# smithlabcode/walt

Hardware: AMD Instinct MI355X
Metric: mapped reads/sec (100 bp single-end, hg19-scale index, -m 6 -b 5000) (higher is better)
Workload: dtype u32

## Files before the change

walt_amd/csrc/core.h:

```cpp
#ifndef WALT_AMD_CORE_H_
#define WALT_AMD_CORE_H_

#include <stdint.h>
#if !defined(__HIPCC__)
#include <stdio.h>
#include <stdlib.h>
#endif

#if defined(__HIPCC__)
#define WALT_HD __host__ __device__ __forceinline__
#else
#define WALT_HD inline
#endif

namespace walt {

#ifndef WALT_SEEDPATTERN
#define WALT_SEEDPATTERN 3
#endif
static_assert(WALT_SEEDPATTERN == 3 || WALT_SEEDPATTERN == 5 || WALT_SEEDPATTERN == 7, "seed pattern 3, 5 or 7");
constexpr uint32_t kPat = WALT_SEEDPATTERN;
constexpr uint32_t kCareW = kPat == 3 ? 1 : (kPat == 5 ? 2 : 4);
constexpr uint32_t kNoCareW = kPat - kCareW;
constexpr uint32_t kKeyWeight = 12;
// ... 1180 lines not shown
  q_of.start_index = iv.start_index; q_of.n_chrom = iv.n_chrom;
  seed_lookup_ex(iv, sv, care, slot, span, seed_len, out, known_good, q_of);
}

WALT_HD Region seed_lookup(const IndexView& iv, const StrandView& sv, const uint32_t* care, uint32_t slot,
                           uint32_t span, uint32_t seed_len) {
  Lookup lk;
  seed_lookup_ex(iv, sv, care, slot, span, seed_len, lk);
  return lk.reg;
}

WALT_HD uint32_t popc32(uint32_t x) {
#if defined(__HIP_DEVICE_COMPILE__)
  return __popc(x);
#else
  return (uint32_t)__builtin_popcount(x);
#endif
}
WALT_HD uint32_t funnel_r(uint32_t lo, uint32_t hi, uint32_t s) {
#if defined(__HIP_DEVICE_COMPILE__)
  return __funnelshift_r(lo, hi, s);
#else
  return (uint32_t)((((uint64_t)hi << 32) | lo) >> s);
#endif
}

constexpr uint32_t tail_care_base_word(uint32_t w) {
  uint32_t m = 0;
  for (uint32_t p = kKeyWeight + kKeyChars; p < kNumCare; ++p) {
    const uint32_t o = care_pos(p);
    if ((o >> 4) == w) m |= 1u << (2 * (o & 15u));
  }
  return m;
}
WALT_HD uint32_t tail_mask_word(uint32_t w, uint32_t lo, uint32_t hi);
template <int W>
WALT_HD uint32_t tail_care_mask_word(uint32_t seed_i, uint32_t cut) {
  constexpr uint32_t b1 = tail_care_base_word(W), b0 = W ? tail_care_base_word(W ? W - 1 : 0) : 0u;
  const uint32_t s = 2 * seed_i;
  const uint32_t m = (b1 << s) | (s ? b0 >> (32 - s) : 0u);
  return m & tail_mask_word(W, 0, cut);
}
WALT_HD uint32_t tail_care_cut(uint32_t seed_i, uint32_t seed_len) {
  return seed_len < kNumCare ? seed_i + care_pos(seed_len) : 0xFFFFu;
}

template <int NW>
WALT_HD uint32_t count_mismatch(const uint32_t* g2, uint32_t gpos, const uint32_t* rd, const uint32_t* mask) {
  const uint32_t* g = g2 + (gpos >> 4);
  uint32_t sh = 2 * (gpos & 15);
  uint32_t mm = 0;
  uint32_t cur = g[0];
#pragma unroll
  for (int w = 0; w < NW; ++w) {
    uint32_t nxt = g[w + 1];
    uint32_t x = funnel_r(cur, nxt, sh) ^ rd[w];
    mm += popc32((x | (x >> 1)) & mask[w]);
    cur = nxt;
  }
  return mm;
}

template <int NW, int W = 0>
WALT_HD void count_mismatch_tail_words(const uint32_t* g, uint32_t sh, const uint32_t* rd, const uint32_t* mask,
                                       uint32_t seed_i, uint32_t cut, uint32_t cur, uint32_t& mm, uint32_t& tmm) {
  if constexpr (W < NW) {
    const uint32_t nxt = g[W + 1];
    const uint32_t x = funnel_r(cur, nxt, sh) ^ rd[W];
    const uint32_t d = x | (x >> 1);
    mm += popc32(d & mask[W]);
    tmm += popc32(d & tail_care_mask_word<W>(seed_i, cut));
    count_mismatch_tail_words<NW, W + 1>(g, sh, rd, mask, seed_i, cut, nxt, mm, tmm);
  }
}
template <int NW>
WALT_HD uint32_t count_mismatch_tail(const uint32_t* g2, uint32_t gpos, const uint32_t* rd, const uint32_t* mask,
                                     uint32_t seed_i, uint32_t cut, uint32_t& tmm) {
  const uint32_t* g = g2 + (gpos >> 4);
  uint32_t mm = 0;
  tmm = 0;
  count_mismatch_tail_words<NW>(g, 2 * (gpos & 15), rd, mask, seed_i, cut, g[0], mm, tmm);
  return mm;
}

template <int NW>
WALT_HD uint32_t count_mismatch_regs(const uint32_t* g , uint32_t sh, const uint32_t* rd, const uint32_t* mask) {
  uint32_t mm = 0;
#if defined(__HIP_DEVICE_COMPILE__)
#pragma unroll
#endif
  for (int w = 0; w < NW; ++w) {
    uint32_t x = funnel_r(g[w], g[w + 1], sh) ^ rd[w];
    mm += popc32((x | (x >> 1)) & mask[w]);
  }
  return mm;
}

template <int NW>
WALT_HD uint32_t count_mismatch_regs2(const uint32_t* g , uint32_t sh, const uint32_t* rd, const uint32_t* mask,
                                      const uint32_t* tmask, uint32_t& tmm) {
  uint32_t mm = 0, t = 0;
#if defined(__HIP_DEVICE_COMPILE__)
#pragma unroll
#endif
  for (int w = 0; w < NW; ++w) {
    const uint32_t x = funnel_r(g[w], g[w + 1], sh) ^ rd[w];
    const uint32_t d = x | (x >> 1);
    mm += popc32(d & mask[w]);
    t += popc32(d & tmask[w]);
  }
  tmm = t;
  return mm;
}

WALT_HD uint32_t align_word(uint32_t cur, uint32_t below, uint32_t sh) {
  return (cur << sh) | ((below >> 1) >> (31u - sh));
}
template <int NW>
WALT_HD void align_read(const uint32_t* rd, const uint32_t* mk, uint32_t sh, uint32_t* rd_a , uint32_t* mk_a ) {
  rd_a[0] = align_word(rd[0], 0u, sh);
  mk_a[0] = align_word(mk[0], 0u, sh);
#if defined(__HIP_DEVICE_COMPILE__)
#pragma unroll
#endif
  for (int w = 1; w < NW; ++w) {
    rd_a[w] = align_word(rd[w], rd[w - 1], sh);
    mk_a[w] = align_word(mk[w], mk[w - 1], sh);
  }
  rd_a[NW] = align_word(0u, rd[NW - 1], sh);
  mk_a[NW] = align_word(0u, mk[NW - 1], sh);
}
template <int NW>
WALT_HD uint32_t count_mismatch_aligned(const uint32_t* g , const uint32_t* rd_a, const uint32_t* mk_a, bool top) {
  uint32_t mm = 0;
#if defined(__HIP_DEVICE_COMPILE__)
#pragma unroll
#endif
  for (int w = 0; w < NW; ++w) {
    const uint32_t x = g[w] ^ rd_a[w];
    mm += popc32((x | (x >> 1)) & mk_a[w]);
  }
  if (top) {
    const uint32_t x = g[NW] ^ rd_a[NW];
    mm += popc32((x | (x >> 1)) & mk_a[NW]);
  }
  return mm;
}
template <int NW>
WALT_HD uint32_t aligned_header_word(uint32_t i, uint32_t cur, uint32_t below, uint32_t sh) {
  const bool first = i == 8u || i == 8u + NW;
  return align_word(cur, first ? 0u : below, i >= 8u ? sh : 0u);
}
WALT_HD uint32_t aligned_header_top(uint32_t last, uint32_t sh) { return align_word(0u, last, sh); }

WALT_HD uint32_t care_mask_word(uint32_t w, uint32_t seed_i, uint32_t p0, uint32_t p1) {
  uint32_t m = 0;
  for (uint32_t p = p0; p < p1; ++p) {
    const uint32_t o = seed_i + care_pos(p);
    if ((o >> 4) == w) m |= 1u << (2 * (o & 15u));
  }
  return m;
}

WALT_HD uint32_t tail_mask_word(uint32_t w, uint32_t lo, uint32_t hi) {
  uint32_t b0 = 16 * w, b1 = b0 + 16;
  uint32_t a = lo > b0 ? lo : b0;
  uint32_t b = hi < b1 ? hi : b1;
  if (a >= b) return 0;
  uint32_t na = a - b0, nb = b - b0;
  uint32_t m = nb == 16 ? 0x55555555u : ((1u << (2 * nb)) - 1u) & 0x55555555u;
  uint32_t below = ((1u << (2 * na)) - 1u);
  return m & ~below;
}
WALT_HD uint32_t mask_table_index(uint32_t seed_i, uint32_t repeats, uint32_t w) {
  return (seed_i * (kMaxRepeats - kMinRepeats + 1) + (repeats - kMinRepeats)) * kMaskWords + w;
}
WALT_HD uint32_t compare_mask_word(const uint32_t* mask_table, uint32_t seed_i, uint32_t repeats,
                                   uint32_t read_len, uint32_t w) {
  uint32_t t = w < kMaskWords ? mask_table[mask_table_index(seed_i, repeats, w)] : 0u;
  return t | tail_mask_word(w, kPat * repeats + seed_i, read_len);
}

struct RegionSummary {
  uint32_t min_mm;
  uint32_t count;
  uint32_t first;
  uint32_t last;
};
WALT_HD RegionSummary summary_empty() { RegionSummary s; s.min_mm = 0xFFFFFFFFu; s.count = 0; s.first = 0; s.last = 0; return s; }
WALT_HD RegionSummary summary_one(uint32_t mm, uint32_t pos) { RegionSummary s; s.min_mm = mm; s.count = 1; s.first = pos; s.last = pos; return s; }
WALT_HD RegionSummary summary_merge(const RegionSummary& a, const RegionSummary& b) {
  const bool has_a = a.count != 0, has_b = b.count != 0;
  const bool take_a = has_a && (!has_b || a.min_mm <= b.min_mm);
  const bool take_b = has_b && (!has_a || b.min_mm <= a.min_mm);
  RegionSummary s;
  s.min_mm = take_a ? a.min_mm : b.min_mm;
  s.count = (take_a ? a.count : 0u) + (take_b ? b.count : 0u);
  s.first = take_a ? a.first : b.first;
  s.last = take_b ? b.last : a.last;
  return s;
}
WALT_HD void fold_region(BestMatch& best, const RegionSummary& s, uint32_t strand_char) {
  if (s.count == 0) return;
  if (s.min_mm < best.mismatch) {
    best.genome_pos = s.last; best.times = s.count; best.strand = strand_char; best.mismatch = s.min_mm;
  } else if (s.min_mm == best.mismatch) {
    uint32_t same = (s.first == best.genome_pos) ? 1u : 0u;
    if (s.count > same) {
      best.times += s.count - same;
      best.genome_pos = s.last;
      best.strand = strand_char;
    }
  }
}

struct HeapEnt {
  uint32_t pos, mms;
};
WALT_HD uint32_t heap_mm(const HeapEnt& e) { return e.mms & 0x7FFFFFFFu; }

template <class H>
WALT_HD void heap_sift_up(H h, uint32_t hole, uint32_t top, HeapEnt v) {
  while (hole > top) {
    uint32_t parent = (hole - 1) / 2;
    if (!(heap_mm(h[parent]) < heap_mm(v))) break;
    h[hole] = h[parent];
    hole = parent;
  }
  h[hole] = v;
}
template <class H>
WALT_HD void heap_push(H h, uint32_t& size, HeapEnt v) {
  heap_sift_up(h, size, 0, v);
  ++size;
}
template <class H>
WALT_HD void heap_adjust(H h, uint32_t hole, uint32_t len, HeapEnt v) {
  const uint32_t top = hole;
  uint32_t child = hole;
  while ((int32_t)child < ((int32_t)len - 1) / 2) {
    child = 2 * (child + 1);
    if (heap_mm(h[child]) < heap_mm(h[child - 1])) --child;
    h[hole] = h[child];
    hole = child;
  }
  if ((len & 1) == 0 && (int32_t)child == ((int32_t)len - 2) / 2) {
    child = 2 * (child + 1);
    h[hole] = h[child - 1];
    hole = child - 1;
  }
  heap_sift_up(h, hole, top, v);
}
template <class H>
WALT_HD HeapEnt heap_pop(H h, uint32_t& size) {
  HeapEnt topv = h[0];
  if (size > 1) {
    HeapEnt v = h[size - 1];
    h[size - 1] = topv;
    heap_adjust(h, 0, size - 1, v);
  }
  --size;
  return topv;
}
template <class H>
WALT_HD void topk_push(H h, uint32_t& size, uint32_t k, HeapEnt v) {
  if (size < k) {
    heap_push(h, size, v);
  } else if (heap_mm(v) < heap_mm(h[0])) {
    heap_pop(h, size);
    heap_push(h, size, v);
  }
}

struct Candidate {
  uint32_t genome_pos;
  uint32_t strand;
  uint32_t mismatch;
};
struct PairResult {
  BestMatch m1, m2;
  uint32_t best_times;
  int32_t frag_len;
  int32_t best_i, best_j;
  uint32_t pair_mm;
  uint32_t pad_[3];
};

WALT_HD void forward_pos(uint32_t gp, uint32_t strand_char, uint32_t chr, uint32_t read_len,
                         const uint32_t* start_index, uint32_t& s, uint32_t& e) {
  uint32_t len = start_index[chr + 1] - start_index[chr];
  uint32_t v = gp - start_index[chr];
  s = strand_char == '+' ? v : len - v - read_len;
  e = s + read_len;
}
WALT_HD void best4single(const Candidate* r, int n, BestMatch& best) {
  for (int i = n - 1; i >= 0; --i) {
    if (r[i].mismatch < best.mismatch) {
      best.genome_pos = r[i].genome_pos; best.times = 1; best.strand = r[i].strand; best.mismatch = r[i].mismatch;
    } else if (r[i].mismatch == best.mismatch) {
      if (best.genome_pos == r[i].genome_pos) continue;
      best.genome_pos = r[i].genome_pos; best.strand = r[i].strand; best.times++;
    } else {
      break;
    }
  }
}
// ... 61 lines not shown
```

walt_amd/csrc/map_se.hip:

```cpp
#include <stdio.h>
#include <stdlib.h>
#include <string.h>

#include "map_common.h"
#include "map_items.h"
#include "group_core.h"

namespace walt {

static __global__ __launch_bounds__(kBlock) void k_ascii_to_2bit(const uint8_t* __restrict__ bases,
                                                                  const uint64_t* __restrict__ offsets, uint32_t n,
                                                                  uint32_t* __restrict__ codes2, uint64_t cap_bytes,
                                                                  uint32_t* __restrict__ err) {
  const uint64_t o0 = offsets[0], all = offsets[n] - o0, total = all < cap_bytes ? all : cap_bytes;
  if (all > cap_bytes && blockIdx.x == 0 && threadIdx.x == 0) atomicAdd(err + 1, 1u);
  const uint8_t* src = bases + o0;
  const uint32_t mis = (uint32_t)(reinterpret_cast<uintptr_t>(src) & 15);
  const uint64_t nwords = (total + 15) / 16;
  uint32_t bad_total = 0;
  for (uint64_t i = (uint64_t)blockIdx.x * blockDim.x + threadIdx.x; i < nwords;
       i += (uint64_t)gridDim.x * blockDim.x) {
    uint32_t qs[4] = {0, 0, 0, 0};
    const uint64_t b0 = 16 * i;
    if (mis == 0 && b0 + 16 <= total) {
// ... 1393 lines not shown
__device__ __forceinline__ const uint4* share_item(const HeavyStage& hs, uint32_t i, uint32_t n_big) {
  constexpr uint32_t Q = item_quads<NW>();
  return i < n_big ? hs.giants + (uint64_t)Q * i : hs.items + (uint64_t)Q * (i - n_big);
}
__device__ __forceinline__ unsigned long long wave_sum_u64(unsigned long long v) {
#pragma unroll
  for (int off = 32; off > 0; off >>= 1) v += __shfl_xor(v, off);
  return v;
}

template <int NW, bool SCATTER>
__global__ __launch_bounds__(kBlock) void k_se_share_bin(HeavyStage hs, SeShare sh) {
  uint32_t n_big, n_all;
  share_counts(hs, n_big, n_all);
  const uint32_t n_grp = n_all < sh.cap ? n_all : sh.cap;
  unsigned long long beyond = 0;
  for (uint32_t i = blockIdx.x * blockDim.x + threadIdx.x; i < (SCATTER ? n_grp : n_all); i += gridDim.x * blockDim.x) {
    const uint4 h = load_global(share_item<NW>(hs, i, n_big));
    if (i < n_grp) {
      const uint32_t bk = group_bucket(group_key(h.x, h.w));
      if constexpr (SCATTER) {
        const uint32_t at = atomicAdd(&sh.cursor[bk], 1u);
        if (at < sh.cap) sh.order[at] = i;
      } else {
        atomicAdd(&sh.count[bk], 1u);
      }
    } else {
      beyond += h.z;
    }
  }
  if constexpr (!SCATTER) {
    if (n_all > n_grp) {
      beyond = wave_sum_u64(beyond);
      if ((threadIdx.x & 63) == 0 && beyond) {
        atomicAdd(&sh.recs[0], beyond);
        atomicAdd(&sh.recs[1], beyond);
      }
    }
  }
}

constexpr uint32_t kShareScanThreads = 1024;
__global__ __launch_bounds__(kShareScanThreads) void k_se_share_scan(SeShare sh) {
  constexpr uint32_t per = kGroupBuckets / kShareScanThreads;
  __shared__ uint32_t part[kShareScanThreads];
  const uint32_t t = threadIdx.x;
  uint32_t s = 0;
  for (uint32_t k = 0; k < per; ++k) s += sh.count[t * per + k];
  part[t] = s;
  __syncthreads();
  for (uint32_t off = 1; off < kShareScanThreads; off <<= 1) {
    const uint32_t v = t >= off ? part[t - off] : 0u;
    __syncthreads();
    part[t] += v;
    __syncthreads();
  }
  uint32_t run = part[t] - s;
  for (uint32_t k = 0; k < per; ++k) {
    sh.cursor[t * per + k] = run;
    run += sh.count[t * per + k];
    sh.count[t * per + k] = 0u;
  }
}

template <int NW>
__global__ __launch_bounds__(kBlock) void k_se_share_cut(HeavyStage hs, SeShare sh) {
  uint32_t n_big, n_all;
  share_counts(hs, n_big, n_all);
  const uint32_t lane = threadIdx.x & 63;
  const uint32_t n_waves = (gridDim.x * blockDim.x) >> 6, wave = (blockIdx.x * blockDim.x + threadIdx.x) >> 6;
  const uint32_t r = sh.r ? sh.r : 1u;
  unsigned long long rec_items = 0, rec_units = 0;
  uint32_t rode = 0;
  const uint32_t end = n_all < sh.cap ? n_all : sh.cap;
  for (uint32_t s = wave * kGroupSlice; s < end; s += n_waves * kGroupSlice) {
    const uint32_t p = s + lane;
    const bool valid = p < end;
    uint32_t item = sh.order[valid ? p : s];
    item = item < n_all ? item : 0u;
    const uint4* it = share_item<NW>(hs, item, n_big);
    const uint4 h0 = load_global(it), h1 = load_global(it + 1);
    const uint64_t key = group_key(h0.x, h0.w);
    const uint32_t size = h0.z, tail = h1.z;
    unsigned long long rem = __ballot(valid);
    uint32_t placed = 0;
    GroupPlace mine = {0u, 0u, 1u, true};
    while (rem) {
      const int ld = (int)__ffsll((long long)rem) - 1;
      const uint64_t lkey = group_key(bcast(h0.x, ld), bcast(h0.w, ld));
      const bool join = (int)lane == ld || group_joins(key, size, tail, lkey, bcast(size, ld), bcast(tail, ld));
      const unsigned long long m = __ballot(join) & rem;
      if ((m >> lane) & 1ull) mine = group_place(m, lane, placed, r);
      placed += (uint32_t)__popcll(m);
      rem &= ~m;
    }
    if (valid) sh.order[s + mine.pos] = item;
    const bool leads = valid && mine.leads, big = size > kBigFirst;
    const unsigned long long mb = __ballot(leads && big), mr = __ballot(leads && !big);
    uint32_t base_b = 0, base_r = 0;
    if (lane == 0) {
      if (mb) base_b = atomicAdd(&sh.ctl[0], (uint32_t)__popcll(mb));
      if (mr) base_r = atomicAdd(&sh.ctl[1], (uint32_t)__popcll(mr));
    }
    base_b = bcast(base_b, 0);
    base_r = bcast(base_r, 0);
    if (leads) {
      const unsigned long long below = (1ull << lane) - 1ull;
      const uint32_t k = big ? base_b + (uint32_t)__popcll(mb & below) : base_r + (uint32_t)__popcll(mr & below);
      if (k < sh.cap) sh.units[big ? k : sh.cap - 1u - k] = make_uint2(mine.unit_n == 1u ? item : s + mine.unit_first, mine.unit_n);
    }
    rec_items += valid ? size : 0u;
    rec_units += leads ? size : 0u;
    rode += (valid && !mine.leads) ? 1u : 0u;
  }
  rec_items = wave_sum_u64(rec_items);
  rec_units = wave_sum_u64(rec_units);
  rode = wave_sum_u32(rode);
  if (lane == 0) {
    if (rec_items) atomicAdd(&sh.recs[0], rec_items);
    if (rec_units) atomicAdd(&sh.recs[1], rec_units);
    if (rode) atomicAdd(&hs.ctl[7], rode);
  }
}

template <int NW, int R>
__global__ __launch_bounds__(kBlock, NW > 7 ? 4 : 5) void k_se_verify_shared(
    IndexView iv, uint32_t strand_base, unsigned long long* __restrict__ stats, HeavyStage hs, SeShare sh, uint32_t b,
    uint32_t* __restrict__ err) {
  static_assert(share_nw<NW>() && item_quads<NW>() <= 8 && R >= 1 && R <= 8, "a unit's headers are fetched by one wavefront load");
  constexpr uint32_t Q = item_quads<NW>();
  {
    ItemQueue q;
    q.items = hs.items; q.ctl = hs.ctl; q.cap = 2 * hs.hcap; q.ovf = err + 2;
    if (blockIdx.x == 0 && threadIdx.x == 0) items_overflow_check(q);
  }
  uint32_t n_big, n_all;
  share_counts(hs, n_big, n_all);
  if (n_all == 0) return;
  const uint32_t n_grp = n_all < sh.cap ? n_all : sh.cap;
  uint32_t nbu = sh.ctl[0], nru = sh.ctl[1];
  nbu = nbu < sh.cap ? nbu : sh.cap;
  nru = nru < sh.cap - nbu ? nru : sh.cap - nbu;
  const uint32_t nu = nbu + nru, n_units = nu + (n_all - n_grp);
  __shared__ uint32_t s_start[kLdsChroms + 1];
  __shared__ uint32_t s_edge[kEdgeWords];
  const bool fits = iv.n_chrom <= kLdsChroms;
  chrom_tab_stage(s_start, iv.start_index, chrom_tab_of(iv.n_chrom));
  const bool has_edge = iv.edge_bits != nullptr;
  if (has_edge)
    for (uint32_t i = threadIdx.x; i < kEdgeWords; i += blockDim.x) s_edge[i] = iv.edge_bits[i];
  __syncthreads();
  const uint32_t n_chrom = iv.n_chrom, top_step = top_step_of(n_chrom);
  const uint32_t lane = threadIdx.x & 63;
  const uint32_t n_waves = (gridDim.x * blockDim.x) >> 6;
  const uint32_t wave = (uint32_t)__builtin_amdgcn_readfirstlane((int)((blockIdx.x * blockDim.x + threadIdx.x) >> 6));
  uint32_t n_verified = 0;
  if (wave < n_units) {
  uint32_t* const cursor = &sh.ctl[2];
  const bool many = n_units >= 32 * n_waves;
  uint32_t batch = many ? n_units / (4 * n_waves) : 2u;
  batch = batch > kVerifyBatchMax ? kVerifyBatchMax : batch;
  const uint32_t first_batch = many ? batch : (uint32_t)((3ull * n_units + 4ull * n_waves - 1) / (4ull * n_waves));
  const uint32_t dealt = n_waves * first_batch;
  auto grab = [&]() {
    uint32_t v = 0;
    if (lane == 0) v = atomicAdd(cursor, batch);
    return v;
  };
  uint32_t b0 = wave, t = 0, stride = n_waves, cur_batch = first_batch, nb_v = 0;
  uint32_t deal = 0;
  if (cur_batch == 1 && dealt < n_units) {
    nb_v = grab();
    deal = 1u;
  }
  auto advance = [&]() __attribute__((always_inline)) -> uint32_t {
    if (deal & 2u) return 0xFFFFFFFFu;
    uint32_t ni;
    if (t + 1 < cur_batch) {
      ++t;
      ni = b0 + t * stride;
    } else {
      b0 = (deal & 1u) ? dealt + bcast(nb_v, 0) : 0xFFFFFFFFu;
      deal = 0u;
      t = 0;
      ni = b0;
      cur_batch = batch;
      stride = 1;
    }
    if (ni >= n_units) {
      deal = 2u;
      return 0xFFFFFFFFu;
    }
    if (t + 1 == cur_batch && dealt < n_units) {
      nb_v = grab();
      deal = 1u;
    }
    return ni;
  };
  auto unit_entry = [&](uint32_t i) __attribute__((always_inline)) -> uint2 {
    const bool on = i < nu;
    const uint64_t at = !on ? 0ull : (i < nbu ? (uint64_t)i : (uint64_t)sh.cap - 1u - (i - nbu));
    uint2 e = load_global(sh.units + at);
    if (!on) e = make_uint2(i < n_units ? sh.cap + (i - nu) : 0u, i < n_units ? 1u : 0u);
    e.x = (uint32_t)__builtin_amdgcn_readfirstlane((int)e.x);
    e.y = (uint32_t)__builtin_amdgcn_readfirstlane((int)e.y);
    e.y = e.y < (uint32_t)R ? e.y : (uint32_t)R;
    return e;
  };
  auto headers = [&](const uint2& e) __attribute__((always_inline)) -> uint4 {
    uint32_t ln = lane;
    asm volatile("" : "+v"(ln));
    const uint32_t rr = ln >> 3, qq = ln & 7u;
    uint32_t item = e.x;
    if (e.y > 1u) {
      const uint32_t p = e.x + (rr < e.y ? rr : 0u);
      item = sh.order[p < sh.cap ? p : 0u];
    }
    item = item < n_all ? item : 0u;
    return load_global(share_item<NW>(hs, item, n_big) + ((rr < e.y && qq < Q) ? qq : 0u));
  };
  auto chrom_bounds_of = [&](uint32_t pos, uint32_t& c_lo, uint32_t& c_hi) {
    if (has_edge && !((s_edge[pos >> (kEdgeBlockShift + 5)] >> ((pos >> kEdgeBlockShift) & 31u)) & 1u)) {
      c_lo = 0; c_hi = 0xFFFFFFFFu;
      return;
    }
    if (fits) {
      const uint32_t chr = chrom_id_steps(s_start, n_chrom, top_step, pos);
      c_lo = s_start[chr]; c_hi = s_start[chr + 1];
    } else {
      walt::chrom_bounds(s_start, iv.start_index, chrom_tab_of(n_chrom), pos, c_lo, c_hi);
    }
  };
  struct Buf { uint4 a, c, e; };
  const uint4 zero = make_uint4(0, 0, 0, 0);
  Buf bx, by;
  bx.a = bx.c = bx.e = by.a = by.c = by.e = zero;
  auto issue = [&](uint32_t fi, uint32_t r0, uint32_t sz, uint32_t base, Buf& y) {
    fi = (uint32_t)__builtin_amdgcn_readfirstlane((int)fi);
    r0 = (uint32_t)__builtin_amdgcn_readfirstlane((int)r0);
    sz = (uint32_t)__builtin_amdgcn_readfirstlane((int)sz);
    const StrandView& sv = iv.s[strand_base + fi];
    const uint32_t k = base + lane;
    const uint64_t rec = (uint64_t)r0 + (k < sz ? k : sz - 1);
    const uint4* rp = reinterpret_cast<const uint4*>(sv.win) + 2 * rec;
    y.a = load_global(rp);
    y.c = load_global(rp + 1);
    if constexpr (NW > 7) y.e = load_global(reinterpret_cast<const uint4*>(sv.win2) + rec);
  };
  auto align_unit = [&](uint4& h) {
    constexpr uint32_t kWordQuads = (8 + 2 * NW + 3) >> 2;
    uint32_t ln = lane;
    asm volatile("" : "+v"(ln));
    const uint32_t q = ln & 7u;
    uint32_t seed_i = (uint32_t)__shfl((int)h.y, (int)((ln & ~7u) | 1u));
    seed_i = seed_i <= kWinLead ? seed_i : 0u;
    const uint32_t sh_read = 2 * (kWinLead - seed_i);
    const uint32_t shv = q < kWordQuads ? sh_read : 0u;
    const uint32_t below = (uint32_t)__shfl((int)h.w, (int)ln - 1);
    uint32_t rd_last = 0;
    if constexpr (NW > 7) rd_last = (uint32_t)__shfl((int)h.w, (int)((ln & ~7u) | (uint32_t)((8 + NW - 1) >> 2)));
    h.w = aligned_header_word<NW>(4 * q + 3, h.w, h.z, shv);
    h.z = aligned_header_word<NW>(4 * q + 2, h.z, h.y, shv);
    h.y = aligned_header_word<NW>(4 * q + 1, h.y, h.x, shv);
    h.x = aligned_header_word<NW>(4 * q + 0, h.x, below, shv);
    if constexpr (NW > 7) {
      constexpr uint32_t kTopQuad = (8 + 2 * NW) >> 2;
      static_assert(((8 + NW - 1) & 3) == 3 && ((8 + 2 * NW) & 3) == 0 && kTopQuad == kWordQuads && kTopQuad < 8,
                    "the last read and mask words are .w components, the top words the .x and .y of the lane behind them");
      h.x = q == kTopQuad ? aligned_header_top(rd_last, sh_read) : h.x;
      h.y = q == kTopQuad ? aligned_header_top(below, sh_read) : h.y;
    }
    asm volatile("" : "+v"(h.x), "+v"(h.y), "+v"(h.z), "+v"(h.w));
  };
  uint2 ue = make_uint2(0u, 0u);
  uint4 hv = zero;
  uint32_t i1 = wave;
  uint2 ue1 = unit_entry(i1);
  uint4 hv1 = headers(ue1);
  uint32_t i2 = advance();
  uint2 ue2 = unit_entry(i2);
  LaneBest acc[R];
  uint32_t strand = 0, size = 1, rec0 = 0, base = 0;
  auto begin = [&]() {
    strand = bcast(hv.x, 0) >> 31; size = bcast(hv.z, 0); rec0 = bcast(hv.w, 0);
    size = size ? size : 1u;
#pragma unroll
    for (int r = 0; r < R; ++r) acc[r] = {0xFFFFFFFFu, 0u, 0u, 0u, 0u, 0u};
    base = 0;
  };
  bool done = false;
  auto step = [&](Buf& x, Buf& y) {
    const bool last = base + 64 >= size;
    const bool hn = i1 != 0xFFFFFFFFu;
    uint32_t n_fi = strand, n_rec0 = rec0, n_size = size;
    const uint32_t n_base = last ? 0u : base + 64;
    if (last && hn) {
      n_fi = bcast(hv1.x, 0) >> 31; n_size = bcast(hv1.z, 0); n_rec0 = bcast(hv1.w, 0);
      n_size = n_size ? n_size : 1u;
    }
    issue(n_fi, n_rec0, n_size, n_base, y);
    const uint32_t k = base + lane;
    const uint32_t pos = x.a.x;
    uint32_t c_lo, c_hi;
    chrom_bounds_of(pos, c_lo, c_hi);
    uint32_t wv[NW + 1];
    const uint32_t first[11] = {x.a.y, x.a.z, x.a.w, x.c.x, x.c.y, x.c.z, x.c.w, NW > 7 ? x.e.x : 0u, NW > 7 ? x.e.y : 0u,
                                NW > 7 ? x.e.z : 0u, NW > 7 ? x.e.w : 0u};
#pragma unroll
    for (int w = 0; w <= NW; ++w) wv[w] = first[w];
#pragma unroll
    for (int r = 0; r < R; ++r) {
      if ((uint32_t)r < ue.y) {
        const uint32_t len = bcast(hv.x, 8 * r + 1), seed_i = bcast(hv.y, 8 * r + 1);
        uint32_t rd[NW + 1], mk[NW + 1];
#pragma unroll
        for (int w = 0; w <= NW; ++w) {
          const int a = w < NW ? 8 + w : 8 + 2 * NW, c = w < NW ? 8 + NW + w : 8 + 2 * NW + 1;
          const uint32_t va = (a & 3) == 0 ? hv.x : (a & 3) == 1 ? hv.y : (a & 3) == 2 ? hv.z : hv.w;
          const uint32_t vc = (c & 3) == 0 ? hv.x : (c & 3) == 1 ? hv.y : (c & 3) == 2 ? hv.z : hv.w;
          rd[w] = (w < NW || NW > 7) ? bcast(va, 8 * r + (a >> 2)) : 0u;
          mk[w] = (w < NW || NW > 7) ? bcast(vc, 8 * r + (c >> 2)) : 0u;
        }
        const uint32_t g = pos - seed_i;
        const bool ok = k < size && (pos - c_lo >= seed_i) && (g + len < c_hi);
        const uint32_t m = count_mismatch_aligned<NW>(wv, rd, mk, NW > 7 && mk[NW] != 0u);
        n_verified += ok ? 1u : 0u;
        lane_best_add(acc[r], k, ok ? g : 0u, ok ? m : 0xFFFFFFFFu);
      }
    }
    if (last) {
#pragma unroll
      for (int r = 0; r < R; ++r) {
        if ((uint32_t)r < ue.y) {
          const uint32_t id = bcast(hv.x, 8 * r), seed_i = bcast(hv.y, 8 * r + 1), tail = bcast(hv.z, 8 * r + 1);
          uint4 res = lane_best_reduce(acc[r]);
          if (tail && size > b) res = make_uint4(0xFFFFFFFFu, 0u, 0u, 0u);
          if (lane == 0) hs.sums[(uint64_t)((id >> 31) ? 1u + seed_i : 0u) * hs.hcap + (id & 0x7FFFFFFFu)] = res;
        }
      }
      if (hn) {
        ue = ue1; hv = hv1;
        align_unit(hv);
        i1 = i2; ue1 = ue2;
        hv1 = headers(ue1);
        i2 = advance();
        ue2 = unit_entry(i2);
        begin();
      } else {
        done = true;
      }
    } else {
      base += 64;
    }
  };
  begin();
  for (;;) {
    step(bx, by);
    if (done) break;
    step(by, bx);
    if (done) break;
  }
  }
  flush_counters({0u, n_verified, 0u}, 0u, stats);
}

#ifndef WALT_LIT_OCC
#define WALT_LIT_OCC 5
#endif
template <int NW, bool LITERAL = true>
__global__ __launch_bounds__(kBlock, NW <= 8 ? WALT_LIT_OCC : 1) void k_map_se_literal(IndexView iv, const uint32_t* __restrict__ codes2,
                                                            const uint64_t* __restrict__ offsets,
                                                            uint32_t* __restrict__ err, uint32_t strand_base,
                                                            uint32_t max_mm,
                                                            uint32_t b, const uint32_t* __restrict__ mask_table,
                                                            BestMatch* __restrict__ out,
                                                            unsigned long long* __restrict__ stats,
                                                            uint32_t* __restrict__ defer_count,
                                                            uint32_t* __restrict__ defer_list,
                                                            uint32_t all_reads, const uint32_t* __restrict__ range = nullptr) {
  uint32_t n_entries = 0;
  if (range != nullptr) {
    const uint32_t lo_entry = range[0];
    n_entries = range[1] > lo_entry ? range[1] - lo_entry : 0u;
    if (n_entries == 0) return;
    defer_list += lo_entry;
  }
  __shared__ BlockShared sh;
  const uint32_t* si = block_prologue(sh, iv, mask_table, strand_base);
  const uint32_t count = all_reads ? all_reads : (range != nullptr ? n_entries : *defer_count);
  MapCounters ctr = {0, 0, 0};
  uint32_t shortv = 0;
  for (uint32_t base = blockIdx.x * blockDim.x; base < count; base += gridDim.x * blockDim.x) {
    const uint32_t i = base + threadIdx.x;
    const bool valid = i < count;
    const uint32_t r = valid ? (all_reads ? i : (defer_list[i] & kDeferMask)) : 0;
    uint32_t len;
#if defined(WALT_DIAG)
    StampsT<true> st;
    stamp_begin(st, g_stage_stamps);
    se_process<NW, LITERAL, true>(iv, sh, si, codes2, offsets, err, r, valid, strand_base, max_mm, b, out,
                                  LITERAL ? nullptr : defer_count, LITERAL ? nullptr : defer_list, ctr, len, 0u, st);
    if (g_stage_stamps_on & 2u) stamp_end(st);
#else
    StampsT<false> st;
    se_process<NW, LITERAL, false>(iv, sh, si, codes2, offsets, err, r, valid, strand_base, max_mm, b, out,
                                   LITERAL ? nullptr : defer_count, LITERAL ? nullptr : defer_list, ctr, len, 0u, st);
#endif
    if (all_reads) shortv += (valid && len < kMinReadLen) ? 2u : 0u;
  }
  flush_counters(ctr, shortv, stats);
}

static inline uint64_t align_up(uint64_t v, uint64_t a) { return (v + a - 1) / a * a; }

uint64_t se_stride(uint32_t n) { return align_up(n ? n : 1, 64); }
constexpr uint32_t kSideCtlWords = 36;
constexpr uint32_t kHeavyCtlWords = 64 * kPat + kSideCtlWords;
static_assert(kHeavyCtlWords % 4 == 0, "the state slots behind the control words are 16-byte aligned");
struct SeGeometry {
  uint32_t hcap;
  uint32_t chunks;
  bool piped;
  uint64_t slot_bytes, heavy_bytes;
};
static uint64_t se_heavy_slot_bytes(uint64_t hcap, int nw) {
  const uint64_t item_q = 2 + (2 * (uint64_t)nw + 3) / 4;
  const uint64_t rd_q = ((uint64_t)nw + 1 + 3) / 4;
  return kPat * hcap * 4 + hcap * (1 + rd_q + kPat + 1) * 16 + (2 * hcap + hcap / 8) * item_q * 16;
}
static SeGeometry se_geometry_for(uint32_t n, int nw, bool pipe, uint64_t chunk_hook) {
  SeGeometry g;
  const uint64_t share = ((uint64_t)n + (pipe ? 7 : 3)) / (pipe ? 8 : 4);
  g.hcap = (uint32_t)align_up(n <= 65536 ? (n ? n : 1) : (share > 65536 ? share : 65536), 64);
  if (chunk_hook > 0 && chunk_hook * 8 >= n) g.hcap = (uint32_t)align_up(chunk_hook, 64);
  const uint32_t k = (uint32_t)(((uint64_t)n + g.hcap - 1) / g.hcap);
  g.piped = pipe && k > 1;
  g.chunks = g.piped ? (k + 1u) & ~1u : k;
  g.slot_bytes = se_heavy_slot_bytes(g.hcap, nw);
  g.heavy_bytes = 16 + kHeavyCtlWords * 4 + (g.piped ? 2 : 1) * g.slot_bytes;
  return g;
}
static uint64_t se_heavy_bytes(uint32_t n, int nw) {
  const uint64_t a = se_geometry_for(n, nw, true, 0).heavy_bytes, c = se_geometry_for(n, nw, false, 0).heavy_bytes;
  return a > c ? a : c;
}
static SeGeometry se_geometry(uint32_t n, int nw, const walt_options& opt) {
  SeGeometry g = se_geometry_for(n, nw, opt.se_pipe != 0, opt.se_heavy_chunk > 0 ? (uint64_t)opt.se_heavy_chunk : 0);
  if (g.heavy_bytes > se_heavy_bytes(n, nw) || g.hcap > (1u << kStageJBits)) g = se_geometry_for(n, nw, opt.se_pipe != 0, 0);
  return g;
}
static uint64_t se_carry_bytes(uint32_t n) { return (uint64_t)kPat * se_stride(n) * 16; }
constexpr uint64_t kShareCtlWords = 4 * kShareRounds;
constexpr uint64_t kShareZeroBytes = 2ull * kGroupBuckets * 4 + kShareCtlWords * 4 + kShareRounds * 2 * 8;
constexpr uint64_t kShareCursorBytes = 2ull * kGroupBuckets * 4;
static uint64_t se_share_slot_bytes(uint64_t cap_items) { return align_up((cap_items & ~1ull) * 12, 16); }
static uint64_t se_share_big_bytes(uint32_t n, int nw) {
  if (nw > 8) return 0;
  uint64_t most = 0;
  for (int pipe = 0; pipe < 2; ++pipe) {
    const SeGeometry g = se_geometry_for(n, nw, pipe != 0, 0);
    const uint64_t v = (g.piped ? 2 : 1) * se_share_slot_bytes(2ull * g.hcap + g.hcap / 8);
    most = v > most ? v : most;
  }
  return most;
}
static uint64_t se_share_bytes(uint32_t n, int nw) { return 32 + se_share_big_bytes(n, nw) + kShareCursorBytes + kShareZeroBytes; }
static uint32_t se_share_cap_for(const SeGeometry& g, uint64_t slot_bytes, long long hook) {
  const uint64_t full = 2ull * g.hcap + g.hcap / 8;
  uint64_t cap = slot_bytes / 12;
  cap = (cap < full ? cap : full) & ~1ull;
  if (hook > 0 && (uint64_t)hook < cap) cap = (uint64_t)hook;
  return (uint32_t)cap;
}

constexpr unsigned kLiteralGrid = 2048;

#if defined(WALT_DIAG)
static uint32_t g_ablate = 0;
static unsigned long long* g_stamps = nullptr;
static void debug_sync(const char* what, hipStream_t stream) {
  static const bool on = getenv("WALT_AMD_SYNC_DEBUG") != nullptr;
  if (!on) return;
  const hipError_t e = hipStreamSynchronize(stream);
  fprintf(stderr, "[walt_amd sync] %s: %s\n", what, hipGetErrorString(e));
}
#else
static void debug_sync(const char*, hipStream_t) {}
#endif

unsigned persistent_grid(const walt_index* idx) {
  return idx->opt.grid > 0 ? (unsigned)idx->opt.grid : (unsigned)idx->n_cu * 8u;
}

struct SeShareArea {
  uint8_t* big = nullptr;
  uint64_t big_bytes = 0;
  uint32_t* zero = nullptr;
};

struct SeWorkspace {
  uint32_t* err;
  unsigned long long* shards;
  uint32_t* defer_count;
  uint32_t* defer_list;
  uint32_t* codes2;
  uint32_t* heavy_area;
  uint4* carry_area;
  SeShareArea share;
// ... 615 lines not shown
```

Baseline: 1.481 billion.

## Stage per-unit read/mask operands in LDS instead of cross-lane broadcasts

When a unit starts, each wave now writes the aligned header words for each read into a per-wave LDS operand area, laid out as interleaved read/mask quads. The inner verify loop then reads them with vector LDS loads instead of issuing many bcast (readlane/shuffle) operations per read per step. Several scheduling values are also made wave-uniform with readfirstlane so they stay in scalar registers. This removes repeated broadcast traffic from the hot loop, at the cost of LDS space, wave-level fences, and added LDS load latency.

Measured after the change: 1.508 billion (median of 6 runs). 1.02x the previous value.

```diff
diff --git a/walt_amd/csrc/core.h b/walt_amd/csrc/core.h
--- a/walt_amd/csrc/core.h
+++ b/walt_amd/csrc/core.h
@@ -1356,6 +1356,22 @@
   return align_word(cur, first ? 0u : below, i >= 8u ? sh : 0u);
 }
 WALT_HD uint32_t aligned_header_top(uint32_t last, uint32_t sh) { return align_word(0u, last, sh); }
+constexpr uint32_t kNoOperand = 0xFFFFFFFFu;
+template <int NW>
+constexpr uint32_t operand_step_words() { return 2u + 2u * NW + (NW > 7 ? 2u : 0u); }
+template <int NW>
+constexpr uint32_t operand_words() { return (operand_step_words<NW>() + 2u + 3u) & ~3u; }
+template <int NW>
+WALT_HD constexpr uint32_t operand_slot(uint32_t i) {
+  return i == 0u ? operand_step_words<NW>()
+         : i == 4u ? 0u
+         : i == 5u ? 1u
+         : i == 6u ? operand_step_words<NW>() + 1u
+         : (i >= 8u && i < 8u + NW) ? 2u + 2u * (i - 8u)
+         : (i >= 8u + NW && i < 8u + 2u * NW) ? 3u + 2u * (i - 8u - NW)
+         : (NW > 7 && (i == 8u + 2u * NW || i == 9u + 2u * NW)) ? 2u + i - 8u
+                                                                 : kNoOperand;
+}
 
 WALT_HD uint32_t care_mask_word(uint32_t w, uint32_t seed_i, uint32_t p0, uint32_t p1) {
   uint32_t m = 0;
diff --git a/walt_amd/csrc/map_se.hip b/walt_amd/csrc/map_se.hip
--- a/walt_amd/csrc/map_se.hip
+++ b/walt_amd/csrc/map_se.hip
@@ -1569,7 +1569,7 @@
   __syncthreads();
   const uint32_t n_chrom = iv.n_chrom, top_step = top_step_of(n_chrom);
   const uint32_t lane = threadIdx.x & 63;
-  const uint32_t n_waves = (gridDim.x * blockDim.x) >> 6;
+  const uint32_t n_waves = (uint32_t)__builtin_amdgcn_readfirstlane((int)((gridDim.x * blockDim.x) >> 6));
   const uint32_t wave = (uint32_t)__builtin_amdgcn_readfirstlane((int)((blockIdx.x * blockDim.x + threadIdx.x) >> 6));
   uint32_t n_verified = 0;
   if (wave < n_units) {
@@ -1577,8 +1577,10 @@
   const bool many = n_units >= 32 * n_waves;
   uint32_t batch = many ? n_units / (4 * n_waves) : 2u;
   batch = batch > kVerifyBatchMax ? kVerifyBatchMax : batch;
-  const uint32_t first_batch = many ? batch : (uint32_t)((3ull * n_units + 4ull * n_waves - 1) / (4ull * n_waves));
-  const uint32_t dealt = n_waves * first_batch;
+  uint32_t first_batch = many ? batch : (uint32_t)((3ull * n_units + 4ull * n_waves - 1) / (4ull * n_waves));
+  batch = (uint32_t)__builtin_amdgcn_readfirstlane((int)batch);
+  first_batch = (uint32_t)__builtin_amdgcn_readfirstlane((int)first_batch);
+  const uint32_t dealt = (uint32_t)__builtin_amdgcn_readfirstlane((int)(n_waves * first_batch));
   auto grab = [&]() {
     uint32_t v = 0;
     if (lane == 0) v = atomicAdd(cursor, batch);
@@ -1689,8 +1691,36 @@
     }
     asm volatile("" : "+v"(h.x), "+v"(h.y), "+v"(h.z), "+v"(h.w));
   };
+  constexpr uint32_t kOpWords = operand_words<NW>(), kOpStep = operand_step_words<NW>();
+  static_assert(kOpStep % 4 == 0 && kOpWords % 4 == 0 && operand_slot<NW>(8) == 2 && operand_slot<NW>(8 + NW) == 3 &&
+                    operand_slot<NW>(8 + 2 * NW - 1) == 2 * NW + 1 && operand_slot<NW>(6) == kOpStep + 1 &&
+                    operand_slot<NW>(8 + 2 * NW + 1) == (NW > 7 ? kOpStep - 1 : kNoOperand),
+                "a step's operands are whole quads, the top words kept only where there are top words");
+  __shared__ __attribute__((aligned(16))) uint32_t s_ops[kBlock / 64][R * kOpWords];
+  uint32_t* const ops = s_ops[threadIdx.x >> 6];
+  auto store_unit = [&](const uint4& h) {
+    uint32_t ln = lane;
+    asm volatile("" : "+v"(ln));
+    const uint32_t rr = ln >> 3, q = ln & 7u;
+    __builtin_amdgcn_fence(__ATOMIC_RELEASE, "wavefront");
+    if (rr < (uint32_t)R) {
+      const uint32_t v[4] = {h.x, h.y, h.z, h.w};
+#pragma unroll
+      for (uint32_t c = 0; c < 4; ++c) {
+        const uint32_t slot = operand_slot<NW>(4 * q + c);
+        if (slot != kNoOperand) ops[rr * kOpWords + slot] = v[c];
+      }
+    }
+    __builtin_amdgcn_fence(__ATOMIC_RELEASE, "wavefront");
+    __builtin_amdgcn_wave_barrier();
+    __builtin_amdgcn_fence(__ATOMIC_ACQUIRE, "wavefront");
+  };
+  typedef uint32_t OpQuad __attribute__((ext_vector_type(4)));
+  constexpr int kOpQuads = (int)(kOpStep / 4);
+  auto load_quad = [&](int r, int j) -> OpQuad {
+    return *reinterpret_cast<const OpQuad*>(ops + (uint32_t)r * kOpWords + 4u * (uint32_t)j);
+  };
   uint2 ue = make_uint2(0u, 0u);
-  uint4 hv = zero;
   uint32_t i1 = wave;
   uint2 ue1 = unit_entry(i1);
   uint4 hv1 = headers(ue1);
@@ -1698,7 +1728,7 @@
   uint2 ue2 = unit_entry(i2);
   LaneBest acc[R];
   uint32_t strand = 0, size = 1, rec0 = 0, base = 0;
-  auto begin = [&]() {
+  auto begin = [&](const uint4& hv) {
     strand = bcast(hv.x, 0) >> 31; size = bcast(hv.z, 0); rec0 = bcast(hv.w, 0);
     size = size ? size : 1u;
 #pragma unroll
@@ -1728,19 +1758,23 @@
 #pragma unroll
     for (int r = 0; r < R; ++r) {
       if ((uint32_t)r < ue.y) {
-        const uint32_t len = bcast(hv.x, 8 * r + 1), seed_i = bcast(hv.y, 8 * r + 1);
-        uint32_t rd[NW + 1], mk[NW + 1];
-#pragma unroll
-        for (int w = 0; w <= NW; ++w) {
-          const int a = w < NW ? 8 + w : 8 + 2 * NW, c = w < NW ? 8 + NW + w : 8 + 2 * NW + 1;
-          const uint32_t va = (a & 3) == 0 ? hv.x : (a & 3) == 1 ? hv.y : (a & 3) == 2 ? hv.z : hv.w;
-          const uint32_t vc = (c & 3) == 0 ? hv.x : (c & 3) == 1 ? hv.y : (c & 3) == 2 ? hv.z : hv.w;
-          rd[w] = (w < NW || NW > 7) ? bcast(va, 8 * r + (a >> 2)) : 0u;
-          mk[w] = (w < NW || NW > 7) ? bcast(vc, 8 * r + (c >> 2)) : 0u;
-        }
+        OpQuad oq[kOpQuads];
+#pragma unroll
+        for (int j = 0; j < kOpQuads; ++j) oq[j] = load_quad(r, j);
+        const uint32_t len = oq[0].x, seed_i = oq[0].y;
         const uint32_t g = pos - seed_i;
         const bool ok = k < size && (pos - c_lo >= seed_i) && (g + len < c_hi);
-        const uint32_t m = count_mismatch_aligned<NW>(wv, rd, mk, NW > 7 && mk[NW] != 0u);
+        uint32_t m = 0;
+#pragma unroll
+        for (int j = 0; j < kOpQuads; ++j) {
+#pragma unroll
+          for (int c = j ? 0 : 2; c < 4; c += 2) {
+            const int w = (4 * j + c - 2) >> 1;
+            const uint32_t x = wv[w] ^ oq[j][c], mk_w = oq[j][c + 1];
+            const uint32_t mm_w = popc32((x | (x >> 1)) & mk_w);
+            if (w < NW || __builtin_amdgcn_readfirstlane((int)mk_w) != 0) m += mm_w;
+          }
+        }
         n_verified += ok ? 1u : 0u;
         lane_best_add(acc[r], k, ok ? g : 0u, ok ? m : 0xFFFFFFFFu);
       }
@@ -1749,20 +1783,22 @@
 #pragma unroll
       for (int r = 0; r < R; ++r) {
         if ((uint32_t)r < ue.y) {
-          const uint32_t id = bcast(hv.x, 8 * r), seed_i = bcast(hv.y, 8 * r + 1), tail = bcast(hv.z, 8 * r + 1);
+          const uint32_t id = ops[r * kOpWords + kOpStep], seed_i = ops[r * kOpWords + 1], tail = ops[r * kOpWords + kOpStep + 1];
           uint4 res = lane_best_reduce(acc[r]);
           if (tail && size > b) res = make_uint4(0xFFFFFFFFu, 0u, 0u, 0u);
           if (lane == 0) hs.sums[(uint64_t)((id >> 31) ? 1u + seed_i : 0u) * hs.hcap + (id & 0x7FFFFFFFu)] = res;
         }
       }
       if (hn) {
-        ue = ue1; hv = hv1;
+        ue = ue1;
+        uint4 hv = hv1;
+        begin(hv);
         align_unit(hv);
+        store_unit(hv);
         i1 = i2; ue1 = ue2;
         hv1 = headers(ue1);
         i2 = advance();
         ue2 = unit_entry(i2);
-        begin();
       } else {
         done = true;
       }
@@ -1770,7 +1806,7 @@
       base += 64;
     }
   };
-  begin();
+  begin(zero);
   for (;;) {
     step(bx, by);
     if (done) break;
```
